# lars-uav/lars-image-processing

Hardware: AMD Instinct MI355X
Metric: Mpixels/sec NDVI+stats on 4096x4096 RGNir tiles; achieved HBM GB/s (higher is better)
Workload: dtype f32

## Files before the change

lars_image_processing_amd/csrc/fused.hip:

```cpp
#include <string.h>

#include "common.h"
#include "device_common.h"
#include "fused_device.h"
#include "wg_device.h"
#include "wb_predict_device.h"

namespace lars {

__global__ __launch_bounds__(256) void k_chan_hist_u8c3(const uint8_t *__restrict__ tiles,
                                                        long long npix, unsigned int *__restrict__ hist)
{
    __shared__ unsigned int s_h[4][3 * 256];
    const int tid = threadIdx.x;
    const int wave = tid >> 6;
    for (int i = tid; i < 4 * 768; i += 256) (&s_h[0][0])[i] = 0;
    __syncthreads();

    const long long tile = blockIdx.y;
    const uint8_t *base = tiles + tile * npix * 3;
    const long long nquads = npix >> 2;
    unsigned int *h = s_h[wave];
    for (long long q = (long long)blockIdx.x * 256 + tid; q < nquads; q += (long long)gridDim.x * 256) {
        const unsigned int *p = reinterpret_cast<const unsigned int *>(base + q * 12);
// ... 165 lines not shown
            const lars_stats *r = rec + t * 3 + k;
            s_sum[tid] = r->sum; s_sq[tid] = r->sumsq;
            cnt += r->count; above += r->above; nans += r->nans;
            mn = fmin(mn, r->min); mx = fmax(mx, r->max);
        }
        __syncthreads();
        const int n = (int)(ntiles - base < 256 ? ntiles - base : 256);
        if (tid == 0) {
            int i = 0;
            if (base == 0) { sum = s_sum[0]; sq = s_sq[0]; i = 1; }
            for (; i < n && (i & 7); ++i) { sum += s_sum[i]; sq += s_sq[i]; }
            for (; i + 8 <= n; i += 8) {
                double a[8], b[8];
#pragma unroll
                for (int j = 0; j < 8; ++j) { a[j] = s_sum[i + j]; b[j] = s_sq[i + j]; }
#pragma unroll
                for (int j = 0; j < 8; ++j) { sum += a[j]; sq += b[j]; }
            }
            for (; i < n; ++i) { sum += s_sum[i]; sq += s_sq[i]; }
        }
        __syncthreads();
    }
    for (int off = 32; off >= 1; off >>= 1) {
        cnt += __shfl_xor(cnt, off); above += __shfl_xor(above, off); nans += __shfl_xor(nans, off);
        mn = fmin(mn, __shfl_xor(mn, off)); mx = fmax(mx, __shfl_xor(mx, off));
    }
    if ((tid & 63) == 0) {
        const int w = tid >> 6;
        s_cnt[w][0] = cnt; s_cnt[w][1] = above; s_cnt[w][2] = nans; s_mn[w] = mn; s_mx[w] = mx;
    }
    __syncthreads();
    lars_stats *o = out + k;
    if (tid == 0) {
        o->sum = sum; o->sumsq = sq;
        o->count = s_cnt[0][0] + s_cnt[1][0] + s_cnt[2][0] + s_cnt[3][0];
        o->above = s_cnt[0][1] + s_cnt[1][1] + s_cnt[2][1] + s_cnt[3][1];
        o->nans = s_cnt[0][2] + s_cnt[1][2] + s_cnt[2][2] + s_cnt[3][2];
        o->min = fmin(fmin(s_mn[0], s_mn[1]), fmin(s_mn[2], s_mn[3]));
        o->max = fmax(fmax(s_mx[0], s_mx[1]), fmax(s_mx[2], s_mx[3]));
        o->threshold = rec[k].threshold; o->index_id = rec[k].index_id; o->reserved = rec[k].reserved;
    }
    if (tid < LARS_HIST_BINS) o->hist[tid] = s_hist[tid];
}

__device__ inline void acc_flush(Acc a, StatsAccView *rec, double (*s_red)[4], int tid)
{
    for (int off = 32; off >= 1; off >>= 1) {
        a.mn = fminf(a.mn, __shfl_xor(a.mn, off));
        a.mx = fmaxf(a.mx, __shfl_xor(a.mx, off));
        a.sum += __shfl_xor(a.sum, off);
        a.sumsq += __shfl_xor(a.sumsq, off);
        a.above += __shfl_xor(a.above, off);
    }
    const int wave = tid >> 6, lane = tid & 63;
    __syncthreads();
    if (lane == 0) {
        s_red[0][wave] = a.sum;
        s_red[1][wave] = a.sumsq;
        s_red[2][wave] = (double)a.above;
        s_red[3][wave] = __builtin_bit_cast(double, ((unsigned long long)f32_key(a.mx) << 32) | f32_key(a.mn));
    }
    __syncthreads();
    if (tid == 0) {
        double sum = 0, sumsq = 0, above = 0;
        unsigned int mnk = 0xFFFFFFFFu, mxk = 0;
        for (int w = 0; w < 4; ++w) {
            sum += s_red[0][w];
            sumsq += s_red[1][w];
            above += s_red[2][w];
            const unsigned long long kk = __builtin_bit_cast(unsigned long long, s_red[3][w]);
            const unsigned int kmn = (unsigned int)kk, kmx = (unsigned int)(kk >> 32);
            mnk = kmn < mnk ? kmn : mnk;
            mxk = kmx > mxk ? kmx : mxk;
        }
        atomicAdd(&rec->sum_fx, (unsigned long long)__double2ll_rn(sum * LARS_FX_SCALE));
        atomicAdd(&rec->sumsq_fx, (unsigned long long)__double2ll_rn(sumsq * LARS_FX_SCALE));
        atomicAdd(&rec->above, (unsigned long long)above);
        atomicMin(&rec->min_key, f64_key((double)key_f32(mnk)));
        atomicMax(&rec->max_key, f64_key((double)key_f32(mxk)));
    }
}


template <typename PIX, unsigned MASK, bool WB, int STATS, int CH = 3, int VERIFY = 0, int POLICY = LOAD_PLAIN>
__global__ __launch_bounds__(256)
__attribute__((amdgpu_waves_per_eu(VERIFY ? 2 : 1, (sizeof(PIX) == 1 && CH == 3 && MASK != 0u && STATS <= 1) ? 3 : 8))) void k_fused_u8c3(FusedParams P, WbGate G)
{
    constexpr bool U16 = sizeof(PIX) == 2;
    static_assert(CH == 3 || (CH == 4 && !U16), "4-channel fast path: uint8 tiles");
    static_assert(!VERIFY || (!U16 && CH == 3 && WB && STATS <= 1), "the verifying form: uint8 RGNir, white balance, at most basic statistics");
    if (VERIFY && G.mode == WB_GATE_MISSED && !wb_gate_open(G, P.npix, blockIdx.y)) return;
    __shared__ unsigned int s_lutv[VERIFY ? 3 * 256 : 1];
    __shared__ unsigned int s_cnt[VERIFY ? 4 * 12 : 1];
    __shared__ uint8_t s_lut[(U16 || VERIFY) ? 16 : 3 * 256];
    __shared__ unsigned int s_thr[U16 ? 3 * 260 : 4];
    __shared__ double s_par[U16 ? 6 : 1];
    constexpr int HIST_COPIES = 16;
    __shared__ unsigned int s_hist_all[HIST_COPIES * 3 * LARS_HIST_BINS];
    __shared__ HistCell<float> s_edges[LARS_HIST_CELLS];
    __shared__ double s_red[4][4];

    const int tid = threadIdx.x;
    unsigned int *const s_hist = s_hist_all + (tid & (HIST_COPIES - 1));
    const unsigned int bx = blockIdx.x, gx = gridDim.x;
    const long long tile = blockIdx.y;
    const long long npix = P.npix;
    const PIX *base = static_cast<const PIX *>(P.tiles) + tile * npix * CH;

    if (WB) {
        if (U16) {
            const uint8_t *blob = P.wb_table + tile * LARS_U16_BLOB_BYTES;
            const unsigned int *thr = reinterpret_cast<const unsigned int *>(blob + LARS_U16_THR_OFFSET);
            const double *par = reinterpret_cast<const double *>(blob + LARS_U16_PAR_OFFSET);
            for (int i = tid; i < 3 * 260; i += 256) s_thr[i] = thr[i];
            if (tid < 6) s_par[tid] = par[tid];
        } else if (VERIFY) {
            const uint8_t *t = P.wb_table + tile * 768;
            const uint8_t *pv = G.predv + tile * 8;
            for (int i = tid; i < 768; i += 256) {
                const unsigned int x = (unsigned int)i & 255u, lo = pv[(i >> 8) * 2], hi = pv[(i >> 8) * 2 + 1];
                s_lutv[i] = ((unsigned int)t[i] << 24) | (x < lo ? 1u : 0u) | (x <= lo ? 1u << 6 : 0u) | (x < hi ? 1u << 12 : 0u) |
                            (x <= hi ? 1u << 18 : 0u);
            }
        } else {
            const uint8_t *t = P.wb_table + tile * 768;
            for (int i = tid; i < 768; i += 256) s_lut[i] = t[i];
        }
    }
    if (STATS >= 2) {
        for (int i = tid; i < HIST_COPIES * 3 * LARS_HIST_BINS; i += 256) s_hist_all[i] = 0;
        hist_cells_init<float>(s_edges, tid);
    }
    if (WB || STATS >= 2) __syncthreads();

    unsigned int vpack[3] = {0u, 0u, 0u};
    unsigned int vcnt[12] = {0u, 0u, 0u, 0u, 0u, 0u, 0u, 0u, 0u, 0u, 0u, 0u};
    auto verify_unpack = [&]() {
#pragma unroll
        for (int c = 0; c < 3; ++c) {
            vcnt[c * 4] += vpack[c] & 63u; vcnt[c * 4 + 1] += (vpack[c] >> 6) & 63u;
            vcnt[c * 4 + 2] += (vpack[c] >> 12) & 63u; vcnt[c * 4 + 3] += (vpack[c] >> 18) & 63u;
            vpack[c] = 0u;
        }
    };
    auto wb_map = [&](unsigned int v, int c) -> unsigned int {
        if (VERIFY) {
            const unsigned int e = s_lutv[c * 256 + v];
            asm("v_add_u32 %0, %0, %1" : "+v"(vpack[c]) : "v"(e));
            return e >> 24;
        }
        if (!U16) return s_lut[c * 256 + v];
        const double y = ((double)v - s_par[2 * c]) * s_par[2 * c + 1];
        int g = (int)y;
        g = g < 0 ? 0 : (g > 255 ? 255 : g);
        const unsigned int *t = s_thr + c * 260;
        g += (v >= t[g + 1] ? 1 : 0) - (v < t[g] ? 1 : 0);
        return (unsigned int)g;
    };

    Acc acc[3];
    acc_init(acc[0]); acc_init(acc[1]); acc_init(acc[2]);

#ifdef LARS_LAB_LAYOUT
    const long long ots = P.out_tile_stride;
#else
    const long long ots = npix;
#endif
    float *const oi0 = P.out_index[0] ? P.out_index[0] + tile * ots : nullptr;
    float *const oi1 = P.out_index[1] ? P.out_index[1] + tile * ots : nullptr;
    float *const oi2 = P.out_index[2] ? P.out_index[2] + tile * ots : nullptr;
    uint8_t *const owb = P.out_wb ? P.out_wb + tile * npix * CH : nullptr;
    uint8_t *const oc0 = P.out_rgba[0] ? P.out_rgba[0] + tile * npix * 4 : nullptr;
    uint8_t *const oc1 = P.out_rgba[1] ? P.out_rgba[1] + tile * npix * 4 : nullptr;
    uint8_t *const oc2 = P.out_rgba[2] ? P.out_rgba[2] + tile * npix * 4 : nullptr;
    const unsigned int *lut0 = reinterpret_cast<const unsigned int *>(P.cmap_lut[0]);
    const unsigned int *lut1 = reinterpret_cast<const unsigned int *>(P.cmap_lut[1]);
    const unsigned int *lut2 = reinterpret_cast<const unsigned int *>(P.cmap_lut[2]);

    const long long nquads = npix >> 2;
    const bool nt_st = (P.flags & 0x20000000u) != 0;
    __amdgpu_buffer_rsrc_t rsrc16;
    if (U16) rsrc16 = __builtin_amdgcn_make_buffer_rsrc(const_cast<PIX *>(base), 0, (int)(nquads * 24), 0x00020000);
    constexpr int NW = U16 ? 6 : 3;

    auto load_quad = [&](long long q, unsigned int (&w)[NW]) {
        if (U16) {
            const unsigned int off = (unsigned int)q * 24u;
            const fu32x4 a4 = stream_load_b128<POLICY>(rsrc16, off, 0);
            const fu32x2 a2 = stream_load_b64<POLICY>(rsrc16, off + 16u, 0);
            w[0] = a4.x; w[1] = a4.y; w[2] = a4.z; w[NW - 3] = a4.w; w[NW - 2] = a2.x; w[NW - 1] = a2.y;
        } else if (CH == 4) {
            const sl_u32x3 a = rgba_quad_to_rgb(
                stream_load_ptr<POLICY>(reinterpret_cast<const sl_u32x4 *>(reinterpret_cast<const uint8_t *>(base) + q * 16)));
            w[0] = a.x; w[1] = a.y; w[2] = a.z;
        } else {
            const unsigned int *p = reinterpret_cast<const unsigned int *>(reinterpret_cast<const uint8_t *>(base) + q * 12);
            w[0] = stream_load_ptr<POLICY>(p); w[1] = stream_load_ptr<POLICY>(p + 1); w[2] = stream_load_ptr<POLICY>(p + 2);
        }
    };
    auto do_quad = [&](long long q, const unsigned int (&w)[NW]) {
        unsigned int b[12];
        if (U16) {
#pragma unroll
            for (int i = 0; i < 6; ++i) { b[2 * i] = w[i % NW] & 0xFFFFu; b[2 * i + 1] = w[i % NW] >> 16; }
        } else {
            const unsigned int w0 = w[0], w1 = w[1], w2 = w[2];
            const unsigned int t[12] = {w0 & 0xFF, (w0 >> 8) & 0xFF, (w0 >> 16) & 0xFF, w0 >> 24,
                                        w1 & 0xFF, (w1 >> 8) & 0xFF, (w1 >> 16) & 0xFF, w1 >> 24,
                                        w2 & 0xFF, (w2 >> 8) & 0xFF, (w2 >> 16) & 0xFF, w2 >> 24};
#pragma unroll
            for (int i = 0; i < 12; ++i) b[i] = t[i];
        }
        if (WB) {
            const bool need_r = (MASK & 1u) || owb || VERIFY, need_g = (MASK & 6u) || owb || VERIFY;
#pragma unroll
            for (int i = 0; i < 12; ++i)
                if (i % 3 == 2 || (i % 3 == 0 && need_r) || (i % 3 == 1 && need_g)) b[i] = wb_map(b[i], i % 3);
            if (owb && CH == 4) {
                *reinterpret_cast<uint4 *>(owb + q * 16) = make_uint4(b[0] | (b[1] << 8) | (b[2] << 16), b[3] | (b[4] << 8) | (b[5] << 16),
                                                                      b[6] | (b[7] << 8) | (b[8] << 16), b[9] | (b[10] << 8) | (b[11] << 16));
            } else if (owb) {
                unsigned int *o = reinterpret_cast<unsigned int *>(owb + q * 12);
                o[0] = b[0] | (b[1] << 8) | (b[2] << 16) | (b[3] << 24);
                o[1] = b[4] | (b[5] << 8) | (b[6] << 16) | (b[7] << 24);
                o[2] = b[8] | (b[9] << 8) | (b[10] << 16) | (b[11] << 24);
            }
        }
        float v0[4], v1[4], v2[4];
#pragma unroll
        for (int px = 0; px < 4; ++px) {
            v0[px] = v1[px] = v2[px] = 0.0f;
            pixel_math<MASK, STATS, false, !U16, HIST_COPIES>((float)b[3 * px], (float)b[3 * px + 1], (float)b[3 * px + 2], 0u,
                                                            v0[px], v1[px], v2[px], acc, s_hist, s_edges);
        }
        if ((MASK & 1u) && oi0) store_plane4(oi0 + q * 4, v0, nt_st);
        if ((MASK & 2u) && oi1) store_plane4(oi1 + q * 4, v1, nt_st);
        if ((MASK & 4u) && oi2) store_plane4(oi2 + q * 4, v2, nt_st);
        if ((MASK & 1u) && oc0)
            *reinterpret_cast<uint4 *>(oc0 + q * 16) = make_uint4(lut0[cmap_index(v0[0])], lut0[cmap_index(v0[1])],
                                                                  lut0[cmap_index(v0[2])], lut0[cmap_index(v0[3])]);
        if ((MASK & 2u) && oc1)
            *reinterpret_cast<uint4 *>(oc1 + q * 16) = make_uint4(lut1[cmap_index(v1[0])], lut1[cmap_index(v1[1])],
                                                                  lut1[cmap_index(v1[2])], lut1[cmap_index(v1[3])]);
        if ((MASK & 4u) && oc2)
            *reinterpret_cast<uint4 *>(oc2 + q * 16) = make_uint4(lut2[cmap_index(v2[0])], lut2[cmap_index(v2[1])],
                                                                  lut2[cmap_index(v2[2])], lut2[cmap_index(v2[3])]);
    };

    constexpr int RUN = (!U16 && CH == 3 && MASK == 7u && STATS == 1) ? (VERIFY ? 12 : 16) : (U16 && MASK == 1u && STATS <= 1) ? 8 : 4;
    const long long nsteps = (nquads + 64 * RUN - 1) / (64 * RUN);
    const long long wstride = (long long)gx * 4;
    const unsigned int lane = (unsigned int)tid & 63u;
    for (long long st = (long long)bx * 4 + (tid >> 6); st < nsteps; st += wstride) {
        const long long q0 = st * (64 * RUN) + lane;
        unsigned int w[RUN][NW];
        if (st * (64 * RUN) + 64 * RUN <= nquads) {
#pragma unroll
            for (int j = 0; j < RUN; ++j) load_quad(q0 + 64 * j, w[j]);
            __builtin_amdgcn_sched_barrier(0);
#pragma unroll
            for (int j = 0; j < RUN; ++j) {
                do_quad(q0 + 64 * j, w[j]);
                __builtin_amdgcn_sched_barrier(0);
            }
        } else {
            for (int j = 0; j < RUN; ++j) {
                const long long q = q0 + 64 * j;
                if (q < nquads) { load_quad(q, w[0]); do_quad(q, w[0]); }
            }
        }
        if (VERIFY) verify_unpack();
    }
    if (bx == 0 && tid < (int)(npix & 3)) {
        const long long i = nquads * 4 + tid;
        unsigned int r = base[i * CH], g = base[i * CH + 1], n = base[i * CH + 2];
        if (WB) { r = wb_map(r, 0); g = wb_map(g, 1); n = wb_map(n, 2); }
        if (WB && owb) {
            owb[i * CH] = (uint8_t)r; owb[i * CH + 1] = (uint8_t)g; owb[i * CH + 2] = (uint8_t)n;
            if (CH == 4) owb[i * CH + 3] = 0;
        }
        float a = 0, bq = 0, c = 0;
        pixel_math<MASK, STATS, false, !U16, HIST_COPIES>((float)r, (float)g, (float)n, 0u, a, bq, c, acc, s_hist, s_edges);
        if ((MASK & 1u) && oi0) oi0[i] = a;
        if ((MASK & 2u) && oi1) oi1[i] = bq;
        if ((MASK & 4u) && oi2) oi2[i] = c;
        if ((MASK & 1u) && oc0) reinterpret_cast<unsigned int *>(oc0)[i] = lut0[cmap_index(a)];
        if ((MASK & 2u) && oc1) reinterpret_cast<unsigned int *>(oc1)[i] = lut1[cmap_index(bq)];
        if ((MASK & 4u) && oc2) reinterpret_cast<unsigned int *>(oc2)[i] = lut2[cmap_index(c)];
    }

    if (VERIFY && G.mode != WB_GATE_MISSED) {
        verify_unpack();
#pragma unroll
        for (int i = 0; i < 12; ++i)
            for (int off = 32; off >= 1; off >>= 1) vcnt[i] += __shfl_xor(vcnt[i], off);
        if ((tid & 63) == 0) {
#pragma unroll
            for (int i = 0; i < 12; ++i) s_cnt[(tid >> 6) * 12 + i] = vcnt[i];
        }
        __syncthreads();
        if (tid < 12) {
            const unsigned int v = s_cnt[tid] + s_cnt[12 + tid] + s_cnt[24 + tid] + s_cnt[36 + tid];
            if (v) atomicAdd(&G.counts[tile * 12 + tid], v);
        }
    }

    if (STATS >= 1) {
        StatsAccView *rec = reinterpret_cast<StatsAccView *>(P.stats + tile * 3);
#pragma unroll
        for (int k = 0; k < 3; ++k)
            if ((MASK & (1u << k)) && (P.mask & (1u << k))) acc_flush(acc[k], rec + k, s_red, tid);
        if (STATS >= 2) {
            __syncthreads();
            for (int i = tid; i < 3 * LARS_HIST_BINS; i += 256) {
                const int k = i / LARS_HIST_BINS;
                unsigned int v = 0;
#pragma unroll
                for (int c = 0; c < HIST_COPIES; ++c) v += s_hist_all[i * HIST_COPIES + ((c + i) & (HIST_COPIES - 1))];
                if ((MASK & (1u << k)) && (P.mask & (1u << k)) && v) atomicAdd(&rec[k].hist[i - k * LARS_HIST_BINS], (unsigned long long)v);
            }
        }
    }
}

template <typename PIX, int NVAL>
__global__ __launch_bounds__(256) void k_fused_generic(FusedParams P)
{
    __shared__ unsigned int s_hist[3 * LARS_HIST_BINS];
    __shared__ HistCell<float> s_edges[LARS_HIST_CELLS];
    __shared__ double s_red[4][4];

    const int tid = threadIdx.x;
    const long long tile = blockIdx.y;
    const long long npix = P.npix;
    const int C = P.channels;
    const unsigned mask = P.mask;
    const bool stats = P.flags & (LARS_F_STATS | LARS_F_HIST | LARS_F_SUMSQ);
    const bool hist = P.flags & (LARS_F_HIST | LARS_F_SUMSQ);
    const bool sumsq = P.flags & LARS_F_SUMSQ;
    const PIX *base = static_cast<const PIX *>(P.tiles) + tile * npix * C;
    const uint8_t *tab = P.wb_table ? P.wb_table + tile * (NVAL == 256 ? 768ll : (long long)LARS_U16_BLOB_BYTES) : nullptr;

    for (int i = tid; i < 3 * LARS_HIST_BINS; i += 256) s_hist[i] = 0;
    hist_cells_init<float>(s_edges, tid);
    __syncthreads();

    Acc acc[3];
    acc_init(acc[0]); acc_init(acc[1]); acc_init(acc[2]);
    float *const oi0 = P.out_index[0] ? P.out_index[0] + tile * npix : nullptr;
    float *const oi1 = P.out_index[1] ? P.out_index[1] + tile * npix : nullptr;
    float *const oi2 = P.out_index[2] ? P.out_index[2] + tile * npix : nullptr;
    uint8_t *const owb = P.out_wb ? P.out_wb + tile * npix * C : nullptr;
    unsigned int *const oc0 = P.out_rgba[0] ? reinterpret_cast<unsigned int *>(P.out_rgba[0]) + tile * npix : nullptr;
    unsigned int *const oc1 = P.out_rgba[1] ? reinterpret_cast<unsigned int *>(P.out_rgba[1]) + tile * npix : nullptr;
    unsigned int *const oc2 = P.out_rgba[2] ? reinterpret_cast<unsigned int *>(P.out_rgba[2]) + tile * npix : nullptr;
    const unsigned int *lut0 = reinterpret_cast<const unsigned int *>(P.cmap_lut[0]);
    const unsigned int *lut1 = reinterpret_cast<const unsigned int *>(P.cmap_lut[1]);
    const unsigned int *lut2 = reinterpret_cast<const unsigned int *>(P.cmap_lut[2]);

    for (long long i = (long long)blockIdx.x * 256 + tid; i < npix; i += (long long)gridDim.x * 256) {
        const PIX *p = base + i * C;
        unsigned int r = p[0], g = p[1], n = p[2];
        if (tab) {
            r = tab[r]; g = tab[NVAL + g]; n = tab[2 * NVAL + n];
            if (owb) {
                uint8_t *o = owb + i * C;
                o[0] = (uint8_t)r; o[1] = (uint8_t)g; o[2] = (uint8_t)n;
                for (int c = 3; c < C; ++c) o[c] = 0;
            }
        }
        float a = 0, b = 0, c = 0;
        if (stats) {
            if (sumsq) pixel_math<7u, 3, true>((float)r, (float)g, (float)n, mask, a, b, c, acc, s_hist, s_edges);
            else if (hist) pixel_math<7u, 2, true>((float)r, (float)g, (float)n, mask, a, b, c, acc, s_hist, s_edges);
            else pixel_math<7u, 1, true>((float)r, (float)g, (float)n, mask, a, b, c, acc, s_hist, s_edges);
        } else {
            pixel_math<7u, 0, true>((float)r, (float)g, (float)n, mask, a, b, c, acc, s_hist, s_edges);
        }
        if ((mask & 1u) && oi0) oi0[i] = a;
        if ((mask & 2u) && oi1) oi1[i] = b;
        if ((mask & 4u) && oi2) oi2[i] = c;
        if ((mask & 1u) && oc0) oc0[i] = lut0[cmap_index(a)];
        if ((mask & 2u) && oc1) oc1[i] = lut1[cmap_index(b)];
        if ((mask & 4u) && oc2) oc2[i] = lut2[cmap_index(c)];
    }
    if (stats) {
        StatsAccView *rec = reinterpret_cast<StatsAccView *>(P.stats + tile * 3);
        for (int k = 0; k < 3; ++k)
            if (mask & (1u << k)) acc_flush(acc[k], rec + k, s_red, tid);
        if (hist) {
            __syncthreads();
            for (int i = tid; i < 3 * LARS_HIST_BINS; i += 256) {
                const int k = i / LARS_HIST_BINS;
                if ((mask & (1u << k)) && s_hist[i])
                    atomicAdd(&rec[k].hist[i - k * LARS_HIST_BINS], (unsigned long long)s_hist[i]);
            }
        }
    }
}

__device__ inline unsigned int mix32(unsigned int x)
{
    x ^= x >> 16; x *= 0x7FEB352Du; x ^= x >> 15; x *= 0x846CA68Bu; x ^= x >> 16;
    return x;
}
// ... 76 lines not shown
        hipLaunchKernelGGL(k_chan_hist_u8c3, grid, dim3(256), 0, s, static_cast<const uint8_t *>(tiles),
                           (long long)npix, hist);
    } else if (dtype == LARS_U8) {
        dim3 grid(blocks_per_tile(npix, ntiles), (unsigned)ntiles);
        hipLaunchKernelGGL((k_chan_hist_generic<uint8_t, 256>), grid, dim3(256), 0, s,
                           static_cast<const uint8_t *>(tiles), (long long)npix, channels, hist);
    } else {
        dim3 grid(blocks_per_tile(npix, ntiles), (unsigned)ntiles);
        hipLaunchKernelGGL((k_chan_hist_generic<uint16_t, 65536>), grid, dim3(256), 0, s,
                           static_cast<const uint16_t *>(tiles), (long long)npix, channels, hist);
    }
    return launch_check("lars_d_channel_hist");
}

extern "C" int lars_d_wb_table(const uint32_t *hist, int64_t ntiles, int64_t npix, int dtype, uint8_t *table,
                               double *percentiles, int rgn_variant, void *stream)
{
    ThreadCtx *c;
    LARS_TRY(ensure_ctx(&c));
    if (!hist || !table || ntiles <= 0 || npix <= 0) return fail(LARS_ERR_INVALID, "lars_d_wb_table: bad arguments");
    if (ntiles > 65535) return fail(LARS_ERR_INVALID, "lars_d_wb_table: ntiles > 65535 per call");
    hipStream_t s = pick_stream(c, stream);
    dim3 grid(3, (unsigned)ntiles);
    if (dtype == LARS_U8)
        hipLaunchKernelGGL((k_wb_table<256>), grid, dim3(256), 0, s, hist, (long long)npix, table, percentiles, rgn_variant, WbGate(),
                           (lars_stats *)nullptr, 0u, (unsigned int *)nullptr);
    else if (dtype == LARS_U16)
        hipLaunchKernelGGL((k_wb_table<65536>), grid, dim3(256), 0, s, hist, (long long)npix, table, percentiles, rgn_variant, WbGate(),
                           (lars_stats *)nullptr, 0u, (unsigned int *)nullptr);
    else
        return fail(LARS_ERR_INVALID, "lars_d_wb_table: dtype");
    return launch_check("lars_d_wb_table");
}

template <typename PIX, unsigned MASK, bool WB, int CH, int POLICY>
static void launch_fast_stats(int stats_mode, dim3 grid, hipStream_t s, const FusedParams &P)
{
    if (stats_mode == 0) hipLaunchKernelGGL((k_fused_u8c3<PIX, MASK, WB, 0, CH, 0, POLICY>), grid, dim3(256), 0, s, P, WbGate());
    else if (stats_mode == 1) hipLaunchKernelGGL((k_fused_u8c3<PIX, MASK, WB, 1, CH, 0, POLICY>), grid, dim3(256), 0, s, P, WbGate());
    else if (stats_mode == 3) hipLaunchKernelGGL((k_fused_u8c3<PIX, MASK, WB, 3, CH, 0, POLICY>), grid, dim3(256), 0, s, P, WbGate());
    else hipLaunchKernelGGL((k_fused_u8c3<PIX, MASK, WB, 2, CH, 0, POLICY>), grid, dim3(256), 0, s, P, WbGate());
}
template <typename PIX, unsigned MASK, int CH, int POLICY>
static void launch_fast_wb(bool wb, int stats_mode, dim3 grid, hipStream_t s, const FusedParams &P)
{
    if (wb) launch_fast_stats<PIX, MASK, true, CH, POLICY>(stats_mode, grid, s, P);
    else launch_fast_stats<PIX, MASK, false, CH, POLICY>(stats_mode, grid, s, P);
}
template <typename PIX, int CH, int POLICY>
static void launch_fast_policy(unsigned mask, bool wb, int stats_mode, dim3 grid, hipStream_t s, const FusedParams &P)
{
    switch (mask) {
    case 0u: hipLaunchKernelGGL((k_fused_u8c3<PIX, 0u, true, 0, CH, 0, POLICY>), grid, dim3(256), 0, s, P, WbGate()); break;
    case 1u: launch_fast_wb<PIX, 1u, CH, POLICY>(wb, stats_mode, grid, s, P); break;
    case 2u: launch_fast_wb<PIX, 2u, CH, POLICY>(wb, stats_mode, grid, s, P); break;
    case 4u: launch_fast_wb<PIX, 4u, CH, POLICY>(wb, stats_mode, grid, s, P); break;
    default: launch_fast_wb<PIX, 7u, CH, POLICY>(wb, stats_mode, grid, s, P); break;
    }
}
template <typename PIX, int CH = 3>
static void launch_fast(unsigned mask, bool wb, int stats_mode, dim3 grid, hipStream_t s, const FusedParams &P, bool default_nt = false)
{
    if (stream_loads_nt(default_nt)) launch_fast_policy<PIX, CH, LOAD_NT>(mask, wb, stats_mode, grid, s, P);
    else launch_fast_policy<PIX, CH, LOAD_PLAIN>(mask, wb, stats_mode, grid, s, P);
}

template <int POLICY>
static void launch_verify_policy(unsigned mask, int stats_mode, dim3 grid, hipStream_t s, const FusedParams &P, const WbGate &G)
{
#define LARS_VERIFY_CASE(M)                                                                                              \
    case M:                                                                                                              \
        if (stats_mode) hipLaunchKernelGGL((k_fused_u8c3<uint8_t, M, true, 1, 3, 1, POLICY>), grid, dim3(256), 0, s, P, G);  \
        else hipLaunchKernelGGL((k_fused_u8c3<uint8_t, M, true, 0, 3, 1, POLICY>), grid, dim3(256), 0, s, P, G);           \
        break;
    switch (mask) {
        LARS_VERIFY_CASE(1u)
        LARS_VERIFY_CASE(2u)
        LARS_VERIFY_CASE(4u)
    default:
        LARS_VERIFY_CASE(7u)
    }
#undef LARS_VERIFY_CASE
}
static void launch_verify(unsigned mask, int stats_mode, dim3 grid, hipStream_t s, const FusedParams &P, const WbGate &G, bool default_nt)
{
    if (stream_loads_nt(default_nt)) launch_verify_policy<LOAD_NT>(mask, stats_mode, grid, s, P, G);
    else launch_verify_policy<LOAD_PLAIN>(mask, stats_mode, grid, s, P, G);
}

namespace lars {
void wb_exact_gated_launch(const uint8_t *tiles, long long ntiles, long long npix, unsigned int *hist, uint8_t *table, double *pcts,
                           int rgn_variant, const WbGate &gate, lars_stats *stats, unsigned int stats_mask, unsigned int *missed, hipStream_t s)
{
    long long want = tuning().blocks_per_tile > 0 ? tuning().blocks_per_tile : (1024 + ntiles - 1) / ntiles;
    const long long cap = (npix / 4 + 1023) / 1024;
    if (want > cap) want = cap;
    if (want < 1) want = 1;
    chan_hist_v2_launch(tiles, npix, hist, dim3((unsigned)want, (unsigned)ntiles), s, 3, gate);
    hipLaunchKernelGGL((k_wb_table<256>), dim3(3, (unsigned)ntiles), dim3(256), 0, s, hist, npix, table, pcts, rgn_variant, gate, stats,
                       stats_mask, missed);
}
}

static int fused_run(const lars_fused_args *a, const lars_wb_verify *v);

extern "C" int lars_d_fused(const lars_fused_args *a) { return fused_run(a, nullptr); }

extern "C" int lars_d_fused_verified(const lars_fused_args *a, const lars_wb_verify *v)
{
    if (!v || !v->scratch || !v->hist || !v->percentiles || v->batch_tiles <= 0 || v->tile_start < 0 || !a || a->ntiles <= 0 ||
        v->tile_start + a->ntiles > v->batch_tiles || !a->wb_table)
        return fail(LARS_ERR_INVALID, "lars_d_fused_verified: bad arguments");
    return fused_run(a, v);
}

static int fused_run(const lars_fused_args *a, const lars_wb_verify *v)
{
    ThreadCtx *c;
    LARS_TRY(ensure_ctx(&c));
    if (!a || !a->tiles || a->ntiles <= 0 || a->npix <= 0 || a->channels < 3)
        return fail(LARS_ERR_INVALID, "lars_d_fused: bad arguments");
    if (a->ntiles > 65535) return fail(LARS_ERR_INVALID, "lars_d_fused: ntiles > 65535 per call");
    if (a->dtype != LARS_U8 && a->dtype != LARS_U16) return fail(LARS_ERR_INVALID, "lars_d_fused: dtype");
    const unsigned mask = a->index_mask & LARS_MASK_ALL;
    if (a->index_mask & ~LARS_MASK_ALL) return fail(LARS_ERR_INVALID, "lars_d_fused: unknown index bits in mask");
    const int stats_mode = (a->flags & LARS_F_SUMSQ) ? 3 : (a->flags & LARS_F_HIST) ? 2 : (a->flags & LARS_F_STATS) ? 1 : 0;
    if (stats_mode && !a->stats) return fail(LARS_ERR_INVALID, "lars_d_fused: stats requested but stats == NULL");
    if (a->out_wb && !a->wb_table) return fail(LARS_ERR_INVALID, "lars_d_fused: out_wb needs wb_table");
    for (int k = 0; k < 3; ++k)
        if (a->out_rgba[k] && !a->cmap_lut[k]) return fail(LARS_ERR_INVALID, "lars_d_fused: out_rgba needs cmap_lut");
    if (mask == 0 && !a->out_wb) return fail(LARS_ERR_INVALID, "lars_d_fused: nothing to do");
    hipStream_t s = pick_stream(c, a->stream);

    FusedParams P;
    P.tiles = a->tiles; P.npix = a->npix; P.channels = a->channels; P.wb_table = a->wb_table;
    for (int k = 0; k < 3; ++k) {
        const bool on = (mask >> k) & 1u;
        P.out_index[k] = on ? a->out_index[k] : nullptr;
        P.out_rgba[k] = on ? a->out_rgba[k] : nullptr;
        P.cmap_lut[k] = a->cmap_lut[k];
    }
    P.out_wb = a->out_wb; P.stats = a->stats; P.mask = mask; P.sel_hist = nullptr; P.sel_win = nullptr; P.sel_win_hist = nullptr; P.sel_below = nullptr;
    P.flags = (a->flags & 7u) | (tuning().nt_stores ? 0x20000000u : 0u);
#ifdef LARS_LAB_LAYOUT
    P.out_tile_stride = a->npix * (tuning().out_stride_planes > 1 ? tuning().out_stride_planes : 1);
#endif

    const long long nrec = a->ntiles * 3;
    const bool raw = (a->flags & LARS_F_RAW) != 0;
    if (stats_mode && !raw)
        hipLaunchKernelGGL(k_stats_init, dim3((unsigned)((nrec + 255) / 256)), dim3(256), 0, s, a->stats, nrec, mask);

    const bool aligned = (reinterpret_cast<uintptr_t>(a->tiles) & 3) == 0 &&
                         (!a->out_wb || (reinterpret_cast<uintptr_t>(a->out_wb) & 3) == 0) &&
                         (!P.out_index[0] || (reinterpret_cast<uintptr_t>(P.out_index[0]) & 15) == 0) &&
                         (!P.out_index[1] || (reinterpret_cast<uintptr_t>(P.out_index[1]) & 15) == 0) &&
                         (!P.out_index[2] || (reinterpret_cast<uintptr_t>(P.out_index[2]) & 15) == 0) &&
                         (!P.out_rgba[0] || (reinterpret_cast<uintptr_t>(P.out_rgba[0]) & 15) == 0) &&
                         (!P.out_rgba[1] || (reinterpret_cast<uintptr_t>(P.out_rgba[1]) & 15) == 0) &&
                         (!P.out_rgba[2] || (reinterpret_cast<uintptr_t>(P.out_rgba[2]) & 15) == 0);
    const unsigned tmask = (mask == 3u || mask == 5u || mask == 6u) ? 7u : mask;
    const bool ch_ok = a->channels == 3 || (a->channels == 4 && a->dtype == LARS_U8 && (reinterpret_cast<uintptr_t>(a->tiles) & 15) == 0 &&
                                            (!a->out_wb || (reinterpret_cast<uintptr_t>(a->out_wb) & 15) == 0));
    const bool fast = ch_ok && aligned && (a->ntiles == 1 || (a->npix & 3) == 0);
    const bool any_out = P.out_wb || P.out_index[0] || P.out_index[1] || P.out_index[2] || P.out_rgba[0] ||
                         P.out_rgba[1] || P.out_rgba[2];
    int impl = tuning().fused_impl;
    if (impl == 0) impl = (any_out && mask != 0u) ? 1 : 2;
    const bool small_tile = (long long)a->npix * 6 < (1ll << 30);
    int &ran = tuning().last_fused_kernel;
    const bool verify = v && fast && a->dtype == LARS_U8 && a->channels == 3 && !(impl >= 2 && small_tile) && a->wb_table && stats_mode <= 1 &&
                        tmask != 0u && a->npix < (1ll << 31);
    WbPredictScratch ps{};
    WbGate G;
    unsigned int *v_hist = nullptr;
    double *v_pcts = nullptr;
    if (v) {
        ps = wb_predict_carve(v->scratch, v->batch_tiles);
        G.pred = ps.pred + v->tile_start; G.predv = ps.predv + v->tile_start * 8; G.counts = ps.counts + v->tile_start * 12;
        v_hist = v->hist + v->tile_start * 768;
        v_pcts = v->percentiles + v->tile_start * 6;
        if (!verify) {
            G.mode = WB_GATE_PREDICTED;
            wb_exact_gated_launch(static_cast<const uint8_t *>(a->tiles), a->ntiles, a->npix, v_hist, const_cast<uint8_t *>(a->wb_table), v_pcts,
                                  v->rgn_variant, G, nullptr, 0u, nullptr, s);
            LARS_HIP_TRY(hipMemsetAsync(ps.pred + v->tile_start, 0, (size_t)a->ntiles * sizeof(unsigned int), s));
        }
    }
    if (verify) {
        dim3 grid(blocks_per_tile(a->npix / 4 + 1, a->ntiles, 256, 32768), (unsigned)a->ntiles);
        const bool three_planes_stats = tmask == 7u && stats_mode == 1 && P.out_index[0] && P.out_index[1] && P.out_index[2];
        G.mode = -1;
        launch_verify(tmask, stats_mode, grid, s, P, G, three_planes_stats);
        G.mode = WB_GATE_MISSED;
        wb_exact_gated_launch(static_cast<const uint8_t *>(a->tiles), a->ntiles, a->npix, v_hist, const_cast<uint8_t *>(a->wb_table), v_pcts,
                              v->rgn_variant, G, stats_mode ? a->stats : nullptr, mask, ps.head + 1, s);
        const dim3 repair_grid(grid.x < 32u ? grid.x : 32u, grid.y);
        launch_verify(tmask, stats_mode, repair_grid, s, P, G, three_planes_stats);
        LARS_HIP_TRY(hipMemsetAsync(ps.pred + v->tile_start, 0, (size_t)a->ntiles * sizeof(unsigned int), s));
        ran = 1;
    } else if (fast && a->dtype == LARS_U8 && a->channels == 3 && impl >= 2 && small_tile) {
        dim3 grid(blocks_per_tile(a->npix / 4 + 1, a->ntiles, fused_v2_threads(any_out || mask == 0u)), (unsigned)a->ntiles);
        fused_v2_launch(tmask, a->wb_table != nullptr, stats_mode, tuning().nt_stores != 0, grid, s, P);
        ran = 2;
    } else if (fast && a->dtype == LARS_U8 && a->channels == 4) {
        dim3 grid(blocks_per_tile(a->npix / 4 + 1, a->ntiles, 256, 32768), (unsigned)a->ntiles);
        launch_fast<uint8_t, 4>(tmask, a->wb_table != nullptr, stats_mode, grid, s, P);
        ran = 5;
    } else if (fast && a->dtype == LARS_U8) {
        dim3 grid(blocks_per_tile(a->npix / 4 + 1, a->ntiles, 256, 32768), (unsigned)a->ntiles);
        const bool three_planes_stats = tmask == 7u && stats_mode == 1 && a->wb_table && P.out_index[0] && P.out_index[1] && P.out_index[2];
        launch_fast<uint8_t>(tmask, a->wb_table != nullptr, stats_mode, grid, s, P, three_planes_stats);
        ran = 1;
    } else if (fast && a->dtype == LARS_U16 && small_tile) {
        dim3 grid(blocks_per_tile(a->npix / 4 + 1, a->ntiles, 256, 32768), (unsigned)a->ntiles);
        launch_fast<uint16_t>(tmask, a->wb_table != nullptr, stats_mode, grid, s, P);
        ran = 3;
    } else {
        dim3 grid(blocks_per_tile(a->npix, a->ntiles), (unsigned)a->ntiles);
        if (a->dtype == LARS_U8) hipLaunchKernelGGL((k_fused_generic<uint8_t, 256>), grid, dim3(256), 0, s, P);
        else hipLaunchKernelGGL((k_fused_generic<uint16_t, 65536>), grid, dim3(256), 0, s, P);
        ran = 4;
    }
    if (stats_mode && !raw)
        hipLaunchKernelGGL(k_stats_finalize, dim3((unsigned)((nrec + 255) / 256)), dim3(256), 0, s, a->stats, nrec, mask,
                           (long long)a->npix);
    return launch_check("lars_d_fused");
}

extern "C" int lars_d_stats_begin(lars_stats *stats, int64_t ntiles, uint32_t index_mask, void *stream)
{
    ThreadCtx *c;
    LARS_TRY(ensure_ctx(&c));
    if (!stats || ntiles <= 0 || (index_mask & ~LARS_MASK_ALL)) return fail(LARS_ERR_INVALID, "lars_d_stats_begin: bad arguments");
    stats_init_launch(stats, ntiles * 3, index_mask & LARS_MASK_ALL, pick_stream(c, stream));
    return launch_check("lars_d_stats_begin");
}
extern "C" int lars_d_stats_end(lars_stats *stats, int64_t ntiles, uint32_t index_mask, int64_t npix, void *stream)
{
    ThreadCtx *c;
    LARS_TRY(ensure_ctx(&c));
    if (!stats || ntiles <= 0 || npix <= 0 || (index_mask & ~LARS_MASK_ALL)) return fail(LARS_ERR_INVALID, "lars_d_stats_end: bad arguments");
    stats_finalize_launch(stats, ntiles * 3, index_mask & LARS_MASK_ALL, (long long)npix, pick_stream(c, stream));
    return launch_check("lars_d_stats_end");
}

extern "C" int lars_d_stats_fold(const lars_stats *tile_records, int64_t ntiles, uint32_t index_mask, lars_stats *out, void *stream)
{
    ThreadCtx *c;
    LARS_TRY(ensure_ctx(&c));
    if (!tile_records || !out || ntiles <= 0 || !(index_mask & LARS_MASK_ALL) || (index_mask & ~LARS_MASK_ALL))
        return fail(LARS_ERR_INVALID, "lars_d_stats_fold: bad arguments");
    hipLaunchKernelGGL(k_stats_fold, dim3(3), dim3(256), 0, pick_stream(c, stream), tile_records, (long long)ntiles,
                       index_mask & LARS_MASK_ALL, out);
    return launch_check("lars_d_stats_fold");
}

extern "C" int lars_d_synth_u8(uint8_t *tiles, int64_t ntiles, int64_t first_tile, int64_t npix, int channels,
                               uint32_t seed, int profile, void *stream)
{
    ThreadCtx *c;
    LARS_TRY(ensure_ctx(&c));
    if (!tiles || ntiles <= 0 || npix <= 0 || channels < 1 || ntiles > 65535)
        return fail(LARS_ERR_INVALID, "lars_d_synth_u8: bad arguments");
    hipStream_t s = pick_stream(c, stream);
    const long long nbytes = (long long)npix * channels;
    dim3 grid(blocks_per_tile((nbytes + 3) / 4, ntiles), (unsigned)ntiles);
    hipLaunchKernelGGL(k_synth_u8, grid, dim3(256), 0, s, tiles, (long long)first_tile, nbytes, channels, seed, profile);
    return launch_check("lars_d_synth_u8");
}

namespace lars {
void stats_init_launch(lars_stats *stats, long long nrec, unsigned int mask, hipStream_t s)
{
    hipLaunchKernelGGL(k_stats_init, dim3((unsigned)((nrec + 255) / 256)), dim3(256), 0, s, stats, nrec, mask);
// ... 7 lines not shown
```

lars_image_processing_amd/csrc/wb_predict.hip:

```cpp
#include "common.h"
#include "device_common.h"
#include "wg_device.h"
#include "wb_predict_device.h"

namespace lars {

constexpr int WBP_GROUPS = 16;
constexpr unsigned int WBP_SEG_BYTES = 4096;

__host__ __device__ inline unsigned int wbp_mix(unsigned int x)
{
    x ^= x >> 16; x *= 0x7FEB352Du; x ^= x >> 15; x *= 0x846CA68Bu; x ^= x >> 16;
    return x;
}
__host__ __device__ inline unsigned int wbp_segment(unsigned int tile, unsigned int i, unsigned int nseg, unsigned int nsample)
{
    const unsigned int start = (unsigned int)(((unsigned long long)i * nseg) / nsample);
    const unsigned int end = (unsigned int)(((unsigned long long)(i + 1) * nseg) / nsample);
    return start + wbp_mix(i * 0x9E3779B9u + tile * 0x85EBCA6Bu + 0x1234567u) % (end - start);
}

template <int POLICY>
__global__ __launch_bounds__(1024) void k_wb_sample_hist(const uint8_t *__restrict__ tiles, long long npix, unsigned int nseg,
                                                         unsigned int nsample, unsigned int *__restrict__ ghist)
{
    __shared__ unsigned int s_h[3 * 256 * 32];
    const int tid = threadIdx.x;
    for (int i = tid; i < 3 * 256 * 32; i += 1024) s_h[i] = 0;
    __syncthreads();

    const unsigned int tile = blockIdx.y, group = blockIdx.x;
    const uint8_t *base = tiles + (long long)tile * npix * 3;
    const __amdgpu_buffer_rsrc_t rsrc =
        __builtin_amdgcn_make_buffer_rsrc(const_cast<uint8_t *>(base), 0, (int)(nseg * WBP_SEG_BYTES), 0x00020000);
    const unsigned int wave = (unsigned int)tid >> 6, lane = (unsigned int)tid & 63u;
    const unsigned int sub = wave >> 2, quarter = wave & 3u;
    const unsigned int per_group = nsample / WBP_GROUPS;
    const unsigned int lane_off = ((unsigned int)tid & 31u) << 2;
    char *hb = reinterpret_cast<char *>(s_h);
#define WBP_ADD(word, shift, choff)                                                                     \
    atomicAdd(reinterpret_cast<unsigned int *>(hb + (choff) + ((((word) >> (shift)) & 0xFFu) << 7) + lane_off), 1u)
    for (unsigned int k0 = sub; k0 < per_group; k0 += 16u) {
        sl_u32x4 w[4];
        unsigned int ph[4];
#pragma unroll
        for (int j = 0; j < 4; ++j) {
            const unsigned int k = k0 + 4u * (unsigned int)j;
            if (k < per_group) {
                const unsigned int seg = wbp_segment(tile, k * WBP_GROUPS + group, nseg, nsample);
                w[j] = stream_load_b128<POLICY>(rsrc, seg * WBP_SEG_BYTES + quarter * 1024u + lane * 16u, 0);
                ph[j] = (seg + quarter + lane) % 3u;
            }
        }
#pragma unroll
        for (int j = 0; j < 4; ++j) {
            if (k0 + 4u * (unsigned int)j < per_group) {
                const unsigned int c0 = ph[j] * 32768u, c1 = ((ph[j] + 1u) % 3u) * 32768u, c2 = ((ph[j] + 2u) % 3u) * 32768u;
                WBP_ADD(w[j].x, 0, c0); WBP_ADD(w[j].x, 8, c1); WBP_ADD(w[j].x, 16, c2); WBP_ADD(w[j].x, 24, c0);
                WBP_ADD(w[j].y, 0, c1); WBP_ADD(w[j].y, 8, c2); WBP_ADD(w[j].y, 16, c0); WBP_ADD(w[j].y, 24, c1);
                WBP_ADD(w[j].z, 0, c2); WBP_ADD(w[j].z, 8, c0); WBP_ADD(w[j].z, 16, c1); WBP_ADD(w[j].z, 24, c2);
                WBP_ADD(w[j].w, 0, c0); WBP_ADD(w[j].w, 8, c1); WBP_ADD(w[j].w, 16, c2); WBP_ADD(w[j].w, 24, c0);
            }
        }
    }
#undef WBP_ADD
    __syncthreads();
    if (tid < 768) {
        const unsigned int *row = s_h + tid * 32;
        unsigned int v = 0;
        for (int j = 0; j < 32; ++j) v += row[(j + tid) & 31];
        ghist[((long long)tile * WBP_GROUPS + group) * 768 + tid] = v;
    }
}

__global__ __launch_bounds__(256) void k_wb_decide(const unsigned int *__restrict__ ghist, int kk, int hook, int rgn_variant,
                                                   unsigned int *__restrict__ head, unsigned int *__restrict__ pred,
                                                   uint8_t *__restrict__ predv, unsigned int *__restrict__ counts,
                                                   uint8_t *__restrict__ table, double *__restrict__ pcts)
{
    __shared__ unsigned int s_g[WBP_GROUPS][768];
    __shared__ unsigned int s_scan[4];
    __shared__ unsigned int s_v[6], s_before[6], s_bin[6], s_n[3];
    __shared__ double s_f[12][WBP_GROUPS];
    __shared__ int s_ok[12];
    __shared__ int s_conf;
    const int tid = threadIdx.x;
    const long long tile = blockIdx.x;
    const unsigned int *g = ghist + tile * WBP_GROUPS * 768;
    for (int i = tid; i < WBP_GROUPS * 768; i += 256) (&s_g[0][0])[i] = g[i];
    __syncthreads();
    for (int c = 0; c < 3; ++c) {
        unsigned int local = 0;
        for (int j = 0; j < WBP_GROUPS; ++j) local += s_g[j][c * 256 + tid];
        unsigned int total = 0;
        const unsigned int before = wg_exscan<256>(local, s_scan, &total);
        if (tid == 0) s_n[c] = total;
        for (int k = 0; k < 2; ++k) {
            long long lo, hi;
            double t;
            wb_mark_ranks(total ? (long long)total : 1, k, lo, hi, t);
            if (local && (unsigned long long)lo >= before && (unsigned long long)lo < (unsigned long long)before + local) {
                s_v[c * 2 + k] = (unsigned int)tid; s_before[c * 2 + k] = before; s_bin[c * 2 + k] = local;
            }
        }
    }
    __syncthreads();
    if (tid < 12 * WBP_GROUPS) {
        const int m = tid / (2 * WBP_GROUPS), e = (tid / WBP_GROUPS) & 1, j = tid % WBP_GROUPS, c = m >> 1;
        const unsigned int *h = &s_g[j][c * 256];
        const unsigned int end = s_n[c] ? s_v[m] + (unsigned int)e : 0u;
        unsigned int cum = 0, all = 0;
        for (unsigned int b = 0; b < 256u; ++b) {
            const unsigned int x = h[(b + (unsigned int)j * 8u) & 255u];
            all += x;
            cum += ((b + (unsigned int)j * 8u) & 255u) < end ? x : 0u;
        }
        s_f[m * 2 + e][j] = all ? (double)cum / (double)all : -1.0;
    }
    __syncthreads();
    if (tid < 12) {
        const int m = tid >> 1, e = tid & 1, c = m >> 1;
        const double q = ((m & 1) == 0 ? 2.0 : 98.0) / 100.0;
        bool ok = s_n[c] != 0u;
        double mean = 0.0;
        for (int j = 0; j < WBP_GROUPS; ++j) { ok = ok && s_f[tid][j] >= 0.0; mean += s_f[tid][j]; }
        mean /= WBP_GROUPS;
        double ss = 0.0;
        for (int j = 0; j < WBP_GROUPS; ++j) ss += (s_f[tid][j] - mean) * (s_f[tid][j] - mean);
        if (ok) {
            const double n = (double)s_n[c];
            double se = sqrt(ss / (double)(WBP_GROUPS * (WBP_GROUPS - 1)));
            const double floor_se = sqrt(q * (1.0 - q) / n);
            if (se < floor_se) se = floor_se;
            const double f = ((double)s_before[m] + (e ? (double)s_bin[m] : 0.0)) / n;
            const double margin = e ? f - q : q - f;
            ok = (e == 0 && s_v[m] == 0u) || (e == 1 && s_v[m] == 255u) || margin >= (double)kk * se;
        }
        s_ok[tid] = ok ? 1 : 0;
    }
    __syncthreads();
    if (tid == 0) {
        bool conf = s_n[0] && s_n[1] && s_n[2];
        for (int i = 0; i < 12; ++i) conf = conf && (s_ok[i] || hook == 3);
        if (conf && hook == 2)
            for (int m = 0; m < 6; ++m) s_v[m] = s_v[m] < 255u ? s_v[m] + 1u : 254u;
// ... 110 lines not shown
```

Measured before the change: 375,100.

## Pipeline WB sample-hist loads through a register ring and skip verify for predicted tiles

Rewrites the white-balance sample histogram kernel so one lane per wave computes the segment indices with a single vector op, then broadcasts them with readlane. A 12-deep ring of 128-bit buffer loads is kept in flight, and sched barriers interleave counting with refills to hide memory latency. The fused kernel now dispatches tiles whose prediction is zero to the non-verifying body, so the verify LUT work is skipped for them. The change also adds lab-only verify forms behind an ifdef, and the extra in-flight loads raise register pressure.

```diff
diff --git a/lars_image_processing_amd/csrc/fused.hip b/lars_image_processing_amd/csrc/fused.hip
--- a/lars_image_processing_amd/csrc/fused.hip
+++ b/lars_image_processing_amd/csrc/fused.hip
@@ -271,17 +271,18 @@
 }
 
 
-template <typename PIX, unsigned MASK, bool WB, int STATS, int CH = 3, int VERIFY = 0, int POLICY = LOAD_PLAIN>
-__global__ __launch_bounds__(256)
-__attribute__((amdgpu_waves_per_eu(VERIFY ? 2 : 1, (sizeof(PIX) == 1 && CH == 3 && MASK != 0u && STATS <= 1) ? 3 : 8))) void k_fused_u8c3(FusedParams P, WbGate G)
+template <typename PIX, unsigned MASK, bool WB, int STATS, int CH, int VERIFY, int POLICY>
+__device__ __forceinline__ void fused_u8c3_body(const FusedParams &P, const WbGate &G)
 {
     constexpr bool U16 = sizeof(PIX) == 2;
     static_assert(CH == 3 || (CH == 4 && !U16), "4-channel fast path: uint8 tiles");
     static_assert(!VERIFY || (!U16 && CH == 3 && WB && STATS <= 1), "the verifying form: uint8 RGNir, white balance, at most basic statistics");
     if (VERIFY && G.mode == WB_GATE_MISSED && !wb_gate_open(G, P.npix, blockIdx.y)) return;
-    __shared__ unsigned int s_lutv[VERIFY ? 3 * 256 : 1];
-    __shared__ unsigned int s_cnt[VERIFY ? 4 * 12 : 1];
-    __shared__ uint8_t s_lut[(U16 || VERIFY) ? 16 : 3 * 256];
+    constexpr bool V_TABLE = VERIFY == 1 || VERIFY >= 3;
+    constexpr bool V_END = VERIFY == 1 || VERIFY >= 4;
+    __shared__ unsigned int s_lutv[V_TABLE ? 3 * 256 : 1];
+    __shared__ unsigned int s_cnt[V_END ? 4 * 12 : 1];
+    __shared__ uint8_t s_lut[(U16 || V_TABLE) ? 16 : 3 * 256];
     __shared__ unsigned int s_thr[U16 ? 3 * 260 : 4];
     __shared__ double s_par[U16 ? 6 : 1];
     constexpr int HIST_COPIES = 16;
@@ -303,7 +304,7 @@
             const double *par = reinterpret_cast<const double *>(blob + LARS_U16_PAR_OFFSET);
             for (int i = tid; i < 3 * 260; i += 256) s_thr[i] = thr[i];
             if (tid < 6) s_par[tid] = par[tid];
-        } else if (VERIFY) {
+        } else if (V_TABLE) {
             const uint8_t *t = P.wb_table + tile * 768;
             const uint8_t *pv = G.predv + tile * 8;
             for (int i = tid; i < 768; i += 256) {
@@ -333,7 +334,7 @@
         }
     };
     auto wb_map = [&](unsigned int v, int c) -> unsigned int {
-        if (VERIFY) {
+        if (V_TABLE) {
             const unsigned int e = s_lutv[c * 256 + v];
             asm("v_add_u32 %0, %0, %1" : "+v"(vpack[c]) : "v"(e));
             return e >> 24;
@@ -401,7 +402,7 @@
             for (int i = 0; i < 12; ++i) b[i] = t[i];
         }
         if (WB) {
-            const bool need_r = (MASK & 1u) || owb || VERIFY, need_g = (MASK & 6u) || owb || VERIFY;
+            const bool need_r = (MASK & 1u) || owb || V_TABLE, need_g = (MASK & 6u) || owb || V_TABLE;
 #pragma unroll
             for (int i = 0; i < 12; ++i)
                 if (i % 3 == 2 || (i % 3 == 0 && need_r) || (i % 3 == 1 && need_g)) b[i] = wb_map(b[i], i % 3);
@@ -458,7 +459,7 @@
                 if (q < nquads) { load_quad(q, w[0]); do_quad(q, w[0]); }
             }
         }
-        if (VERIFY) verify_unpack();
+        if (V_TABLE) verify_unpack();
     }
     if (bx == 0 && tid < (int)(npix & 3)) {
         const long long i = nquads * 4 + tid;
@@ -478,7 +479,14 @@
         if ((MASK & 4u) && oc2) reinterpret_cast<unsigned int *>(oc2)[i] = lut2[cmap_index(c)];
     }
 
-    if (VERIFY && G.mode != WB_GATE_MISSED) {
+    if (V_TABLE && !V_END) {
+        verify_unpack();
+        unsigned int x = 0;
+#pragma unroll
+        for (int i = 0; i < 12; ++i) x ^= vcnt[i];
+        if (x == 0xFFFFFFFFu) G.counts[tile * 12] = x;
+    }
+    if (V_END && G.mode != WB_GATE_MISSED) {
         verify_unpack();
 #pragma unroll
         for (int i = 0; i < 12; ++i)
@@ -510,6 +518,19 @@
             }
         }
     }
+}
+
+template <typename PIX, unsigned MASK, bool WB, int STATS, int CH = 3, int VERIFY = 0, int POLICY = LOAD_PLAIN>
+__global__ __launch_bounds__(256)
+__attribute__((amdgpu_waves_per_eu(VERIFY ? 2 : 1, (sizeof(PIX) == 1 && CH == 3 && MASK != 0u && STATS <= 1) ? 3 : 8))) void k_fused_u8c3(FusedParams P, WbGate G)
+{
+    if constexpr (VERIFY == 1) {
+        if (G.mode != WB_GATE_MISSED && G.pred[blockIdx.y] == 0u) {
+            fused_u8c3_body<PIX, MASK, WB, STATS, CH, 0, POLICY>(P, G);
+            return;
+        }
+    }
+    fused_u8c3_body<PIX, MASK, WB, STATS, CH, VERIFY, POLICY>(P, G);
 }
 
 template <typename PIX, int NVAL>
@@ -752,6 +773,27 @@
     }
 #undef LARS_VERIFY_CASE
 }
+#ifdef LARS_LAB_VERIFY
+static int lab_verify_form()
+{
+    const char *e = getenv("LARS_LAB_VERIFY_FORM");
+    return e && *e ? atoi(e) : -1;
+}
+static bool lab_verify_launch(int form, dim3 grid, hipStream_t s, const FusedParams &P, const WbGate &G)
+{
+#define LARS_LAB_FORM(V) \
+    case V: hipLaunchKernelGGL((k_fused_u8c3<uint8_t, 7u, true, 1, 3, V, LOAD_NT>), grid, dim3(256), 0, s, P, G); return true;
+    switch (form) {
+        LARS_LAB_FORM(0)
+        LARS_LAB_FORM(1)
+        LARS_LAB_FORM(2)
+        LARS_LAB_FORM(3)
+        LARS_LAB_FORM(4)
+    default: return false;
+    }
+#undef LARS_LAB_FORM
+}
+#endif
 static void launch_verify(unsigned mask, int stats_mode, dim3 grid, hipStream_t s, const FusedParams &P, const WbGate &G, bool default_nt)
 {
     if (stream_loads_nt(default_nt)) launch_verify_policy<LOAD_NT>(mask, stats_mode, grid, s, P, G);
@@ -861,6 +903,12 @@
         dim3 grid(blocks_per_tile(a->npix / 4 + 1, a->ntiles, 256, 32768), (unsigned)a->ntiles);
         const bool three_planes_stats = tmask == 7u && stats_mode == 1 && P.out_index[0] && P.out_index[1] && P.out_index[2];
         G.mode = -1;
+#ifdef LARS_LAB_VERIFY
+        if (three_planes_stats && lab_verify_launch(lab_verify_form(), grid, s, P, G)) {
+            ran = 1;
+            return launch_check("lars_d_fused (laboratory form)");
+        }
+#endif
         launch_verify(tmask, stats_mode, grid, s, P, G, three_planes_stats);
         G.mode = WB_GATE_MISSED;
         wb_exact_gated_launch(static_cast<const uint8_t *>(a->tiles), a->ntiles, a->npix, v_hist, const_cast<uint8_t *>(a->wb_table), v_pcts,
diff --git a/lars_image_processing_amd/csrc/wb_predict.hip b/lars_image_processing_amd/csrc/wb_predict.hip
--- a/lars_image_processing_amd/csrc/wb_predict.hip
+++ b/lars_image_processing_amd/csrc/wb_predict.hip
@@ -20,6 +20,8 @@
     return start + wbp_mix(i * 0x9E3779B9u + tile * 0x85EBCA6Bu + 0x1234567u) % (end - start);
 }
 
+constexpr int WBP_RING = 12;
+constexpr int WBP_CHUNK = 48;
 template <int POLICY>
 __global__ __launch_bounds__(1024) void k_wb_sample_hist(const uint8_t *__restrict__ tiles, long long npix, unsigned int nseg,
                                                          unsigned int nsample, unsigned int *__restrict__ ghist)
@@ -33,34 +35,56 @@
     const uint8_t *base = tiles + (long long)tile * npix * 3;
     const __amdgpu_buffer_rsrc_t rsrc =
         __builtin_amdgcn_make_buffer_rsrc(const_cast<uint8_t *>(base), 0, (int)(nseg * WBP_SEG_BYTES), 0x00020000);
-    const unsigned int wave = (unsigned int)tid >> 6, lane = (unsigned int)tid & 63u;
+    const unsigned int wave = (unsigned int)__builtin_amdgcn_readfirstlane(tid >> 6), lane = (unsigned int)tid & 63u;
     const unsigned int sub = wave >> 2, quarter = wave & 3u;
     const unsigned int per_group = nsample / WBP_GROUPS;
+    const unsigned int nloads = per_group > sub ? (per_group - sub + 3u) / 4u : 0u;
     const unsigned int lane_off = ((unsigned int)tid & 31u) << 2;
+    const unsigned int voff = quarter * 1024u + lane * 16u;
+    const unsigned int pl = (quarter + lane) % 3u;
+    const unsigned int o0 = pl * 32768u, o1 = ((pl + 1u) % 3u) * 32768u, o2 = ((pl + 2u) % 3u) * 32768u;
     char *hb = reinterpret_cast<char *>(s_h);
 #define WBP_ADD(word, shift, choff)                                                                     \
     atomicAdd(reinterpret_cast<unsigned int *>(hb + (choff) + ((((word) >> (shift)) & 0xFFu) << 7) + lane_off), 1u)
-    for (unsigned int k0 = sub; k0 < per_group; k0 += 16u) {
-        sl_u32x4 w[4];
-        unsigned int ph[4];
+    auto count = [&](const sl_u32x4 &w, unsigned int seg) {
+        const unsigned int s3 = seg % 3u;
+        const unsigned int c0 = s3 == 0u ? o0 : s3 == 1u ? o1 : o2, c1 = s3 == 0u ? o1 : s3 == 1u ? o2 : o0,
+                           c2 = s3 == 0u ? o2 : s3 == 1u ? o0 : o1;
+        WBP_ADD(w.x, 0, c0); WBP_ADD(w.x, 8, c1); WBP_ADD(w.x, 16, c2); WBP_ADD(w.x, 24, c0);
+        WBP_ADD(w.y, 0, c1); WBP_ADD(w.y, 8, c2); WBP_ADD(w.y, 16, c0); WBP_ADD(w.y, 24, c1);
+        WBP_ADD(w.z, 0, c2); WBP_ADD(w.z, 8, c0); WBP_ADD(w.z, 16, c1); WBP_ADD(w.z, 24, c2);
+        WBP_ADD(w.w, 0, c0); WBP_ADD(w.w, 8, c1); WBP_ADD(w.w, 16, c2); WBP_ADD(w.w, 24, c0);
+    };
+    for (unsigned int cb = 0; cb < nloads; cb += (unsigned int)WBP_CHUNK) {
+        const unsigned int cn = nloads - cb < (unsigned int)WBP_CHUNK ? nloads - cb : (unsigned int)WBP_CHUNK;
+        unsigned int segv = 0u;
+        if (lane < cn) segv = wbp_segment(tile, (sub + 4u * (cb + lane)) * WBP_GROUPS + group, nseg, nsample);
+        auto seg_of = [&](unsigned int i) {
+            return (unsigned int)__builtin_amdgcn_readlane((int)segv, (int)i);
+        };
+        const unsigned int rounds = cn / (unsigned int)WBP_RING;
+        if (rounds > 0u) {
+            sl_u32x4 w[WBP_RING];
 #pragma unroll
-        for (int j = 0; j < 4; ++j) {
-            const unsigned int k = k0 + 4u * (unsigned int)j;
-            if (k < per_group) {
-                const unsigned int seg = wbp_segment(tile, k * WBP_GROUPS + group, nseg, nsample);
-                w[j] = stream_load_b128<POLICY>(rsrc, seg * WBP_SEG_BYTES + quarter * 1024u + lane * 16u, 0);
-                ph[j] = (seg + quarter + lane) % 3u;
+            for (int j = 0; j < WBP_RING; ++j) w[j] = stream_load_b128<POLICY>(rsrc, voff, seg_of((unsigned int)j) * WBP_SEG_BYTES);
+            for (unsigned int r = 0; r + 1u < rounds; ++r) {
+#pragma unroll
+                for (int j = 0; j < WBP_RING; ++j) {
+                    count(w[j], seg_of(r * (unsigned int)WBP_RING + (unsigned int)j));
+                    __builtin_amdgcn_sched_barrier(0);
+                    w[j] = stream_load_b128<POLICY>(rsrc, voff, seg_of((r + 1u) * (unsigned int)WBP_RING + (unsigned int)j) * WBP_SEG_BYTES);
+                    __builtin_amdgcn_sched_barrier(0);
+                }
             }
-        }
 #pragma unroll
-        for (int j = 0; j < 4; ++j) {
-            if (k0 + 4u * (unsigned int)j < per_group) {
-                const unsigned int c0 = ph[j] * 32768u, c1 = ((ph[j] + 1u) % 3u) * 32768u, c2 = ((ph[j] + 2u) % 3u) * 32768u;
-                WBP_ADD(w[j].x, 0, c0); WBP_ADD(w[j].x, 8, c1); WBP_ADD(w[j].x, 16, c2); WBP_ADD(w[j].x, 24, c0);
-                WBP_ADD(w[j].y, 0, c1); WBP_ADD(w[j].y, 8, c2); WBP_ADD(w[j].y, 16, c0); WBP_ADD(w[j].y, 24, c1);
-                WBP_ADD(w[j].z, 0, c2); WBP_ADD(w[j].z, 8, c0); WBP_ADD(w[j].z, 16, c1); WBP_ADD(w[j].z, 24, c2);
-                WBP_ADD(w[j].w, 0, c0); WBP_ADD(w[j].w, 8, c1); WBP_ADD(w[j].w, 16, c2); WBP_ADD(w[j].w, 24, c0);
+            for (int j = 0; j < WBP_RING; ++j) {
+                count(w[j], seg_of((rounds - 1u) * (unsigned int)WBP_RING + (unsigned int)j));
+                __builtin_amdgcn_sched_barrier(0);
             }
+        }
+        for (unsigned int i = rounds * (unsigned int)WBP_RING; i < cn; ++i) {
+            const unsigned int seg = seg_of(i);
+            count(stream_load_b128<POLICY>(rsrc, voff, seg * WBP_SEG_BYTES), seg);
         }
     }
 #undef WBP_ADD
```

Measured after the change: 387,500, median of 6. +3.3%, better.
